# apple/ml-pgdvs

Measured on AMD Instinct MI355X. Metric: novel-view frames/s at 1080p x 24 src frames; achieved HBM GB/s vs gfx950 peak, higher is better.
Workload: dtype f32

## Files before the change

ml-pgdvs_amd/csrc/raster.hip:

```cpp
#include <cstdlib>

#include "common.h"
#include "raster_cam.h"

namespace pgdvs {

constexpr int kTile = 16;

struct TileBox {
  int tx0, tx1, ty0, ty1;
};

__device__ __forceinline__ TileBox tile_box(const RasterCam &rc, float3 p, float radius, int H,
                                            int W, int ntx, int nty) {
  TileBox b;
  b.tx0 = 1;
  b.tx1 = 0;
  b.ty0 = 1;
  b.ty1 = 0;
  if (!(p.z >= 0.0f) || !isfinite(p.x) || !isfinite(p.y)) return b;
  float offx = rc.range_x / 2.0f, offy = rc.range_y / 2.0f;
  float xc = (float)(W - 1) - ((p.x + offx) * (float)W - offx) / rc.range_x;
  float yc = (float)(H - 1) - ((p.y + offy) * (float)H - offy) / rc.range_y;
  float rpx = radius * (float)W / rc.range_x + 0.0625f;
// ... 157 lines not shown
  for (int64_t i = lo + threadIdx.x; i < hi; i += kBinThreads) {
    const float cur[3] = {nxt[0], nxt[1], nxt[2]};
    if (i + kBinThreads < hi && i + kBinThreads < n) {
      const float *X = pts + (i + kBinThreads) * pts_stride;
      nxt[0] = X[0]; nxt[1] = X[1]; nxt[2] = X[2];
    }
    TileBox b;
    b.tx0 = 1; b.tx1 = 0; b.ty0 = 1; b.ty1 = 0;
    float pz = 0.0f;
    if (i < n) {
      float3 p = point_to_ndc(rc, cur[0], cur[1], cur[2]);
      b = tile_box(rc, p, radius, H, W, ntx, nty);
      pz = p.z + 0.0f;
    }
    int nx = 2, ny = 2;
    if (!box2) {
      nx = wave_max_i32_scalar(b.tx1 - b.tx0 + 1);
      ny = wave_max_i32_scalar(b.ty1 - b.ty0 + 1);
    }
    for (int jy = 0; jy < ny; ++jy)
      for (int jx = 0; jx < nx; ++jx) {
        int tx = b.tx0 + jx, ty = b.ty0 + jy;
        int t = (tx <= b.tx1 && ty <= b.ty1) ? ty * ntx + tx : -1;
        if (tile_bound != nullptr && t >= 0 && pz > tile_bound[t]) t = -1;
        if (local)
          wave_tile_count_lds(s_tab, t);
        else
          wave_tile_count(tile_count, t);
      }
  }
  if (local) {
    __syncthreads();
    for (int t = threadIdx.x; t < ntiles; t += kBinThreads) {
      const int v = s_tab[t];
      if (v) __hip_atomic_fetch_add(&tile_count[t], v, __ATOMIC_RELAXED, __HIP_MEMORY_SCOPE_AGENT);
    }
  }
}

__global__ void __launch_bounds__(1024)
raster_scan_kernel(const int32_t *__restrict__ counts, int n, int32_t *__restrict__ offsets, const int32_t *__restrict__ run_flag) {
  __shared__ int wave_sums[1024 / kWave];
  if (run_flag != nullptr && *run_flag == 0) return;
  constexpr int kPer = 8;
  const int lane = threadIdx.x & 63, wave = threadIdx.x >> 6;
  int carry = 0;
  for (int start = 0; start < n; start += 1024 * kPer) {
    const int i0 = start + (int)threadIdx.x * kPer;
    int v[kPer], s = 0;
#pragma unroll
    for (int k = 0; k < kPer; ++k) {
      v[k] = i0 + k < n ? counts[i0 + k] : 0;
      s += v[k];
    }
    int x = s;
    for (int off = 1; off < 64; off <<= 1) {
      const int y = __shfl_up(x, off, 64);
      if (lane >= off) x += y;
    }
    if (lane == 63) wave_sums[wave] = x;
    __syncthreads();
    int run = carry + x - s, total = 0;
#pragma unroll
    for (int w = 0; w < 1024 / kWave; ++w) {
      if (w < wave) run += wave_sums[w];
      total += wave_sums[w];
    }
#pragma unroll
    for (int k = 0; k < kPer; ++k) {
      if (i0 + k < n) offsets[i0 + k] = run;
      run += v[k];
    }
    carry += total;
    __syncthreads();
  }
  if (threadIdx.x == 0) offsets[n] = carry;
}

constexpr int kFillPer = 4;
constexpr int kFillThreads = 256;
constexpr int kFillMaxSpan = 2;

constexpr int kFillTouchCap = 1024;

__device__ __forceinline__ int wave_tile_reserve_lds(int *s_tab, int t, unsigned short *s_touch, int *s_ntouch) {
  const int lane = threadIdx.x & 63;
  RunInfo r = wave_runs(t);
  int base = 0;
  if (r.is_leader && t >= 0) {
    base = atomicAdd(&s_tab[t], r.length);
    if (base == 0) {
      const int at = atomicAdd(s_ntouch, 1);
      if (at < kFillTouchCap) s_touch[at] = (unsigned short)t;
    }
  }
  base = __shfl(base, r.leader, 64);
  return base + (lane - r.leader);
}

template <int kSlots>
__global__ void __launch_bounds__(kFillThreads)
raster_fill_kernel(const float *__restrict__ pts, int64_t pts_stride, int64_t n_host, const int64_t *__restrict__ n_dev,
                   const float *__restrict__ cam, float radius, int H, int W, int ntx, int nty,
                   const int32_t *__restrict__ offsets,
                   int32_t *__restrict__ cursor, float4 *__restrict__ lists,
                   int64_t list_capacity, const float *__restrict__ tile_bound, int64_t gate_rows,
                   int seg, int32_t *__restrict__ overflow, int32_t *__restrict__ status, const int32_t *__restrict__ run_flag) {
  __shared__ int s_tab[kSlots];
  __shared__ unsigned short s_touch[kFillTouchCap];
  __shared__ int s_ntouch;
  static_assert(kSlots <= 65536, "tile numbers in the touched list are 16 bits wide");
  int n_touched = kFillTouchCap + 1;
  if (run_flag != nullptr && *run_flag == 0) return;
  int64_t n = n_dev ? *n_dev : n_host;
  if (status != nullptr && blockIdx.x == 0 && threadIdx.x == 0) *status = n > n_host ? 1 : (n < 0 ? 2 : 0);
  if (seg > 0 && blockIdx.x == 0 && threadIdx.x == 0) overflow[1] = 1;
  n = n > n_host ? n_host : (n < 0 ? 0 : n);
  if (n < gate_rows) tile_bound = nullptr;
  RasterCam rc = make_raster_cam(cam, H, W);
  const int ntiles = ntx * nty;
  const bool local = ntiles <= kSlots && tile_box_within_2x2(rc, radius, H, W);
  constexpr int64_t kChunk = (int64_t)kFillThreads * kFillPer;
  for (int64_t c0 = (int64_t)blockIdx.x * kChunk; c0 < n; c0 += (int64_t)gridDim.x * kChunk) {
    int t0[kFillPer], span[kFillPer];
    float ex[kFillPer], ey[kFillPer], ez[kFillPer];
#pragma unroll
    for (int u = 0; u < kFillPer; ++u) {
      const int64_t i = c0 + (int64_t)u * kFillThreads + threadIdx.x;
      const float *X = pts + (i < n ? i : n - 1) * pts_stride;
      ex[u] = X[0];
      ey[u] = X[1];
      ez[u] = X[2];
    }
    if (local) {
      if (n_touched <= kFillTouchCap) {
        for (int k = threadIdx.x; k < n_touched; k += kFillThreads) s_tab[s_touch[k]] = 0;
      } else {
        for (int t = threadIdx.x; t < ntiles; t += kFillThreads) s_tab[t] = 0;
      }
      if (threadIdx.x == 0) s_ntouch = 0;
      __syncthreads();
    }
#pragma unroll
    for (int u = 0; u < kFillPer; ++u) {
      const int64_t i = c0 + (int64_t)u * kFillThreads + threadIdx.x;
      TileBox b;
      b.tx0 = 1; b.tx1 = 0; b.ty0 = 1; b.ty1 = 0;
      if (i < n) {
        const float3 q = point_to_ndc(rc, ex[u], ey[u], ez[u]);
        b = tile_box(rc, q, radius, H, W, ntx, nty);
        ex[u] = q.x;
        ey[u] = q.y;
        ez[u] = q.z + 0.0f;
      }
      t0[u] = b.ty0 * ntx + b.tx0;
      span[u] = (b.tx1 - b.tx0 + 1) | ((b.ty1 - b.ty0 + 1) << 16);
      if (tile_bound != nullptr && local) {
        unsigned behind = 0;
#pragma unroll
        for (int jy = 0; jy < kFillMaxSpan; ++jy)
#pragma unroll
          for (int jx = 0; jx < kFillMaxSpan; ++jx)
            if (jx < (span[u] & 0xff) && jy < (span[u] >> 16) && ez[u] > tile_bound[t0[u] + jy * ntx + jx]) behind |= 1u << (8 + jy * 2 + jx);
        span[u] |= (int)behind;
      }
    }
    if (local) {
      unsigned rank[kFillPer][kFillMaxSpan];
#pragma unroll
      for (int u = 0; u < kFillPer; ++u) {
#pragma unroll
        for (int jy = 0; jy < kFillMaxSpan; ++jy) {
          rank[u][jy] = 0;
#pragma unroll
          for (int jx = 0; jx < kFillMaxSpan; ++jx) {
            const int t = (jx < (span[u] & 0xff) && jy < (span[u] >> 16) && !((span[u] >> (8 + jy * 2 + jx)) & 1))
                              ? t0[u] + jy * ntx + jx : -1;
            rank[u][jy] |= ((unsigned)wave_tile_reserve_lds(s_tab, t, s_touch, &s_ntouch) & 0xffffu) << (16 * jx);
          }
        }
      }
      static_assert(kChunk <= 65536, "ranks are packed in 16 bits");
      __syncthreads();
      n_touched = s_ntouch;
      if (n_touched <= kFillTouchCap) {
        for (int kb = threadIdx.x; kb < n_touched; kb += kFillThreads * 4) {
          int t[4], v[4], r[4];
#pragma unroll
          for (int k = 0; k < 4; ++k) {
            const int idx = kb + k * kFillThreads;
            t[k] = idx < n_touched ? (int)s_touch[idx] : -1;
            v[k] = t[k] >= 0 ? s_tab[t[k]] : 0;
          }
#pragma unroll
          for (int k = 0; k < 4; ++k) {
            r[k] = 0;
            if (t[k] >= 0) {
              if (seg > 0) {
                const int at = atomicAdd(&cursor[t[k]], v[k]);
                if (at + v[k] > seg) atomicOr(overflow, 1);
                r[k] = t[k] * seg + at;
              } else {
                r[k] = offsets[t[k]] + atomicAdd(&cursor[t[k]], v[k]);
              }
            }
          }
#pragma unroll
          for (int k = 0; k < 4; ++k)
            if (t[k] >= 0) s_tab[t[k]] = r[k];
        }
      } else
      for (int tb = threadIdx.x; tb < ntiles; tb += kFillThreads * 4) {
        int v[4], r[4];
#pragma unroll
        for (int k = 0; k < 4; ++k) {
          const int t = tb + k * kFillThreads;
          v[k] = t < ntiles ? s_tab[t] : 0;
        }
#pragma unroll
        for (int k = 0; k < 4; ++k) {
          const int t = tb + k * kFillThreads;
          if (seg > 0) {
            const int at = v[k] ? atomicAdd(&cursor[t], v[k]) : 0;
            if (at + v[k] > seg) atomicOr(overflow, 1);
            r[k] = t * seg + at;
          } else {
            r[k] = v[k] ? offsets[t] + atomicAdd(&cursor[t], v[k]) : 0;
          }
        }
#pragma unroll
        for (int k = 0; k < 4; ++k)
          if (v[k]) s_tab[tb + k * kFillThreads] = r[k];
      }
      __syncthreads();
#pragma unroll
      for (int u = 0; u < kFillPer; ++u) {
        const int64_t i = c0 + (int64_t)u * kFillThreads + threadIdx.x;
        const float4 ent = make_float4(ex[u], ey[u], __int_as_float((int)i), ez[u]);
#pragma unroll
        for (int jy = 0; jy < kFillMaxSpan; ++jy)
#pragma unroll
          for (int jx = 0; jx < kFillMaxSpan; ++jx)
            if (jx < (span[u] & 0xff) && jy < (span[u] >> 16) && !((span[u] >> (8 + jy * 2 + jx)) & 1)) {
              const int t = t0[u] + jy * ntx + jx;
              const int64_t pos = (int64_t)s_tab[t] + (int)((rank[u][jy] >> (16 * jx)) & 0xffffu);
              if (pos < (seg > 0 ? (int64_t)(t + 1) * seg : list_capacity)) lists[pos] = ent;
            }
      }
      __syncthreads();
    } else {
#pragma unroll
      for (int u = 0; u < kFillPer; ++u) {
        const int64_t i = c0 + (int64_t)u * kFillThreads + threadIdx.x;
        const float4 ent = make_float4(ex[u], ey[u], __int_as_float((int)i), ez[u]);
        const int nx = wave_max_i32_scalar(span[u] & 0xffff), ny = wave_max_i32_scalar(span[u] >> 16);
        for (int jy = 0; jy < ny; ++jy)
          for (int jx = 0; jx < nx; ++jx) {
            int t = (jx < (span[u] & 0xffff) && jy < (span[u] >> 16)) ? t0[u] + jy * ntx + jx : -1;
            if (tile_bound != nullptr && t >= 0 && ez[u] > tile_bound[t]) t = -1;
            const int slot = wave_tile_reserve(cursor, t);
            if (t >= 0) {
              if (seg > 0) {
                if (slot < seg)
                  lists[(int64_t)t * seg + slot] = ent;
                else
                  atomicOr(overflow, 1);
              } else {
                const int64_t pos = (int64_t)offsets[t] + slot;
                if (pos < list_capacity) lists[pos] = ent;
              }
            }
          }
      }
    }
  }
}

template <int K>
struct TopK {
  unsigned long long key[K];
  static constexpr unsigned long long kEmpty = ~0ull;
  __device__ __forceinline__ void init() {
#pragma unroll
    for (int k = 0; k < K; ++k) key[k] = kEmpty;
  }
  __device__ __forceinline__ bool has(int k) const { return key[k] != kEmpty; }
  __device__ __forceinline__ int id(int k) const { return (int)(unsigned)(key[k] & 0xffffffffull); }
  __device__ __forceinline__ float z(int k) const { return __uint_as_float((unsigned)(key[k] >> 32)); }
  __device__ __forceinline__ void insert_below_last(unsigned long long kk) {
    bool c[K];
#pragma unroll
    for (int k = 0; k < K - 1; ++k) c[k] = kk < key[k];
    c[K - 1] = true;
#pragma unroll
    for (int k = K - 1; k > 0; --k) key[k] = c[k - 1] ? key[k - 1] : (c[k] ? kk : key[k]);
    key[0] = c[0] ? kk : key[0];
  }
};

constexpr int kSortCap = 2048;
constexpr int kSortCapLong = 4096;
constexpr int kSortBuckets = 1024;
constexpr int kSortMaxBucket = 64;

template <int K>
__device__ __forceinline__ void rank_insert(float (&key)[K], float r) {
#pragma unroll
  for (int k = K - 1; k > 0; --k) key[k] = __builtin_amdgcn_fmed3f(key[k - 1], key[k], r);
  asm("v_min_f32 %0, %1, %2" : "=v"(key[0]) : "v"(key[0]), "v"(r));
}

__device__ __forceinline__ float readlane_f(float v, int lane) {
  return __int_as_float(__builtin_amdgcn_readlane(__float_as_int(v), lane));
}

template <int K, int kCap, bool kFrag>
__global__ void __launch_bounds__(256, kCap <= kSortCap ? (kFrag ? 4 : 5) : 2)
raster_tile_kernel(const float4 *__restrict__ lists, const int32_t *__restrict__ offsets, int64_t list_capacity,
                   const float4 *__restrict__ seg_lists, const int32_t *__restrict__ seg_count, int seg,
                   const int32_t *__restrict__ seg_overflow, int pass,
                   const float *__restrict__ feat, int64_t feat_stride, float radius, int H, int W,
                   int ntx, int nty, int tiles_per_xcd, int64_t *__restrict__ idx_out,
                   float *__restrict__ zbuf_out, float *__restrict__ dist_out,
                   float *__restrict__ rgb_out, int rgb_planar, float *__restrict__ mask_out, int32_t *__restrict__ stats) {
  constexpr int kSortPerThread = kCap / 256;
  __shared__ uint2 s_buf[kCap];
  uint2 *s_kz = s_buf;
  float2 *s_xy = reinterpret_cast<float2 *>(s_buf);
  __shared__ unsigned s_id[kCap];
  __shared__ unsigned s_zr[kFrag ? kCap : 1];
  __shared__ float4 s_wave[4][68];
  unsigned *s_cnt = reinterpret_cast<unsigned *>(&s_wave[0][0]);
  static_assert(kSortBuckets * 4 <= 4 * 68 * 16, "the counters alias the strips");
  static_assert(kCap * (kFrag ? 16 : 12) + 4 * 68 * 16 + 128 <= (kCap <= kSortCap ? (kFrag ? 40960 : 32768) : 81920),
                "four / five (two) workgroups per CU");
  static_assert(kCap % 256 == 0 && kCap <= 4096, "every thread owns kCap / 256 entries; positions are packed in 12 bits");
  __shared__ unsigned s_red[12];
  __shared__ int s_flag;
  const int ntiles = ntx * nty;
  (void)tiles_per_xcd;
  const int tile = blockIdx.x;
  if (tile >= ntiles) return;
  const int ty = tile / ntx, tx = tile - ty * ntx;
  const int tid = threadIdx.x, lane = tid & 63, wave = tid >> 6;
  const int lx = (wave & 1) * 8 + (lane & 7), ly = (wave >> 1) * 8 + (lane >> 3);
  const int xi = tx * kTile + lx, yi = ty * kTile + ly;
  const bool inside = xi < W && yi < H;
  const float range_x = W > H ? 2.0f * (float)W / (float)H : 2.0f;
  const float range_y = H > W ? 2.0f * (float)H / (float)W : 2.0f;
  const float xf = inside ? pix_to_ndc(W - 1 - xi, W, range_x) : __builtin_nanf("");
  const float yf = pix_to_ndc(H - 1 - yi, H, range_y);
  const float r2 = radius * radius;
  const int qx0 = tx * kTile + (wave & 1) * 8, qy0 = ty * kTile + (wave >> 1) * 8;
  const float margin = radius * 1.001f + 1e-6f;
  const float bx_hi = pix_to_ndc(W - 1 - qx0, W, range_x) + margin;
  const float bx_lo = pix_to_ndc(W - 1 - (qx0 + 7), W, range_x) - margin;
  const float by_hi = pix_to_ndc(H - 1 - qy0, H, range_y) + margin;
  const float by_lo = pix_to_ndc(H - 1 - (qy0 + 7), H, range_y) - margin;
  const bool direct = seg > 0 && *seg_overflow == 0;
  int64_t beg, end;
  if (direct) {
    beg = (int64_t)tile * seg;
    end = beg + seg_count[tile];
  } else {
    beg = offsets[tile];
    end = offsets[tile + 1];
    if (end > list_capacity) end = list_capacity;
  }
  const int64_t n64 = end > beg ? end - beg : 0;
  const float4 *__restrict__ L = (direct ? seg_lists : lists) + beg;

  bool has[K];
  int rid[K];
  float rz[K], rd2[K];
#pragma unroll
  for (int k = 0; k < K; ++k) {
    has[k] = false;
    rid[k] = -1;
    rz[k] = -1.0f;
    rd2[k] = -1.0f;
  }

  if ((pass == 1 && n64 > kSortCap) || (pass == 2 && n64 <= kSortCap)) return;
  bool sorted_path = n64 > 0 && n64 <= kCap;
  if (sorted_path) {
    const int n = (int)n64;
    float4 ent[kSortPerThread];
#pragma unroll
    for (int k = 0; k < kSortPerThread; ++k) {
      const int e = tid + k * 256;
      ent[k] = L[e < n ? e : n - 1];
    }
    unsigned zmn = 0xffffffffu, zmx = 0u;
#pragma unroll
    for (int k = 0; k < kSortPerThread; ++k) {
      const unsigned zb = __float_as_uint(ent[k].w);
      zmn = zb < zmn ? zb : zmn;
      zmx = zb > zmx ? zb : zmx;
    }
#pragma unroll
    for (int off = 32; off > 0; off >>= 1) {
      const unsigned a = __shfl_xor(zmn, off, 64), b = __shfl_xor(zmx, off, 64);
      zmn = a < zmn ? a : zmn;
      zmx = b > zmx ? b : zmx;
    }
    if (lane == 0) {
      s_red[wave] = zmn;
      s_red[4 + wave] = zmx;
    }
#pragma unroll
    for (int j = 0; j < kSortBuckets / 256; ++j) s_cnt[tid + j * 256] = 0u;
    if (tid == 0) s_flag = 0;
    __syncthreads();
#pragma unroll
    for (int w = 0; w < 4; ++w) {
      zmn = s_red[w] < zmn ? s_red[w] : zmn;
      zmx = s_red[4 + w] > zmx ? s_red[4 + w] : zmx;
    }
    const float scale = (float)kSortBuckets / ((float)(zmx - zmn) + 1.0f);
    unsigned pos[kSortPerThread];
#pragma unroll
    for (int k = 0; k < kSortPerThread; ++k) {
      pos[k] = 0u;
      if (k * 256 < n) {
        const int e = tid + k * 256;
        if (e < n) {
          const unsigned zb = __float_as_uint(ent[k].w);
          unsigned b = (unsigned)((float)(zb - zmn) * scale);
          b = b < (unsigned)kSortBuckets - 1u ? b : (unsigned)kSortBuckets - 1u;
          pos[k] = (b << 12) | atomicAdd(&s_cnt[b], 1u);
        }
      }
    }
    __syncthreads();
    {
      unsigned c[kSortBuckets / 256], tot = 0u, mx = 0u;
#pragma unroll
      for (int j = 0; j < kSortBuckets / 256; ++j) {
        c[j] = s_cnt[tid * (kSortBuckets / 256) + j];
        mx = c[j] > mx ? c[j] : mx;
        tot += c[j];
      }
      if (mx > (unsigned)kSortMaxBucket) s_flag = 1;
      unsigned incl = tot;
#pragma unroll
      for (int off = 1; off < 64; off <<= 1) {
        const unsigned y = __shfl_up(incl, off, 64);
        if (lane >= off) incl += y;
      }
      if (lane == 63) s_red[8 + wave] = incl;
      __syncthreads();
      unsigned base = incl - tot;
#pragma unroll
      for (int w = 0; w < 4; ++w)
        if (w < wave) base += s_red[8 + w];
#pragma unroll
      for (int j = 0; j < kSortBuckets / 256; ++j) {
        s_cnt[tid * (kSortBuckets / 256) + j] = base;
        base += c[j];
      }
    }
    __syncthreads();
    sorted_path = s_flag == 0;
    if (!sorted_path && tid == 0) atomicAdd(&stats[0], 1);
    if (sorted_path) {
#pragma unroll
      for (int k = 0; k < kSortPerThread; ++k) {
        if (k * 256 < n) {
          const int e = tid + k * 256;
          if (e < n) {
            const float4 q = ent[k];
            const unsigned b = pos[k] >> 12;
            const unsigned p = s_cnt[b] + (pos[k] & 0xfffu);
            s_kz[p] = make_uint2(__float_as_uint(q.w), __float_as_uint(q.z));
            pos[k] = (b << 12) | p;
          }
        }
      }
      __syncthreads();
#pragma unroll
      for (int k = 0; k < kSortPerThread; ++k) {
        if (k * 256 < n) {
          const int e = tid + k * 256;
          if (e < n) {
            const unsigned b = pos[k] >> 12, p = pos[k] & 0xfffu;
            const unsigned bs = s_cnt[b], be = b + 1u < (unsigned)kSortBuckets ? s_cnt[b + 1u] : (unsigned)n;
            const uint2 me = s_kz[p];
            unsigned r = bs;
            uint2 o[4];
#pragma unroll
            for (int j = 0; j < 4; ++j) o[j] = s_kz[bs + j < (unsigned)n ? bs + j : (unsigned)n - 1u];
#pragma unroll
            for (int j = 0; j < 4; ++j)
              r += (bs + j < be) & ((o[j].x < me.x) | ((o[j].x == me.x) & (o[j].y < me.y))) ? 1u : 0u;
            for (unsigned j = bs + 4u; j < be; ++j) {
              const uint2 oj = s_kz[j];
              r += (oj.x < me.x) | ((oj.x == me.x) & (oj.y < me.y)) ? 1u : 0u;
            }
            pos[k] = r;
          }
        }
      }
      __syncthreads();
#pragma unroll
      for (int k = 0; k < kSortPerThread; ++k) {
        if (k * 256 < n) {
          const int e = tid + k * 256;
          if (e < n) {
            const float4 q = ent[k];
            s_xy[pos[k]] = make_float2(q.x, q.y);
            s_id[pos[k]] = __float_as_uint(q.z);
            if (kFrag) s_zr[pos[k]] = __float_as_uint(q.w);
          }
        }
      }
      __syncthreads();
      float key[K];
#pragma unroll
      for (int k = 0; k < K; ++k) key[k] = __builtin_inff();
      float4 *strip = s_wave[wave];
      for (int base = 0; base < n; base += 64) {
        const unsigned long long open = __ballot(inside && key[K - 1] == __builtin_inff());
        if (open == 0ull) break;
        const int r_lo = __builtin_ctzll(open) >> 3, r_hi = (63 - __builtin_clzll(open)) >> 3;
        unsigned cols = (unsigned)(open | (open >> 32));
        cols |= cols >> 16;
        cols = (cols | (cols >> 8)) & 0xffu;
        const int c_lo = __builtin_ctz(cols), c_hi = 31 - __builtin_clz(cols);
        const float ox_hi = readlane_f(xf, __builtin_ctzll(open & (0x0101010101010101ull << c_lo)));
        const float ox_lo = readlane_f(xf, __builtin_ctzll(open & (0x0101010101010101ull << c_hi)));
        const float oy_hi = readlane_f(yf, r_lo * 8), oy_lo = readlane_f(yf, r_hi * 8);
        const int e = base + lane;
        const float2 c = s_xy[e < n ? e : 0];
        const float ex = fmaxf(fmaxf(ox_lo - c.x, c.x - ox_hi), 0.0f), ey = fmaxf(fmaxf(oy_lo - c.y, c.y - oy_hi), 0.0f);
        const bool in = e < n && ex * ex + ey * ey <= margin * margin;
        const unsigned long long mask = __ballot(in);
        if (!mask) continue;
        const int cnt = (int)__popcll(mask);
        if (in) strip[__popcll(mask & ((1ull << lane) - 1ull))] = make_float4(c.x, c.y, (float)e, 0.f);
        if (lane < 3) strip[cnt + lane] = make_float4(__builtin_inff(), __builtin_inff(), __builtin_inff(), 0.f);
        __builtin_amdgcn_wave_barrier();
        float4 p[4], pn[4];
#pragma unroll
        for (int u = 0; u < 4; ++u) p[u] = strip[u];
        for (int j = 0; j < cnt; j += 4) {
#pragma unroll
          for (int u = 0; u < 4; ++u) pn[u] = strip[(j + 4 + u) & 63];
#pragma unroll
          for (int u = 0; u < 4; ++u) {
            const float dx = p[u].x - xf, dy = p[u].y - yf;
            const float d2 = dx * dx + dy * dy;
            rank_insert<K>(key, d2 < r2 ? p[u].z : __builtin_inff());
          }
#pragma unroll
          for (int u = 0; u < 4; ++u) p[u] = pn[u];
        }
        __builtin_amdgcn_wave_barrier();
      }
#pragma unroll
      for (int k = 0; k < K; ++k) {
        if (key[k] != __builtin_inff()) {
          const int r = (int)key[k];
          const float2 c = s_xy[r];
          const float dx = c.x - xf, dy = c.y - yf;
          has[k] = true;
          rid[k] = (int)s_id[r];
          rz[k] = kFrag ? __uint_as_float(s_zr[kFrag ? r : 0]) : 0.0f;
          rd2[k] = dx * dx + dy * dy;
        }
      }
    }
  }
  if (!sorted_path && n64 > 0) {
    __syncthreads();
    float4 *s_pt = reinterpret_cast<float4 *>(s_xy);
    TopK<K> q;
    q.init();
    for (int64_t base = 0; base < n64; base += 256) {
      const int64_t e = base + tid;
      __syncthreads();
      if (e < n64) s_pt[tid] = L[e];
      __syncthreads();
      const int m = (int)((n64 - base) < 256 ? (n64 - base) : 256);
      for (int sub = 0; sub < m; sub += 64) {
        const int zcull = wave_max_i32_scalar(inside ? (q.has(K - 1) ? (int)(q.key[K - 1] >> 32) : 0x7fffffff) : 0);
        const float4 c = s_pt[(sub + lane) & 255];
        const bool hit = (sub + lane) < m && c.x >= bx_lo && c.x <= bx_hi && c.y >= by_lo && c.y <= by_hi &&
                         __float_as_int(c.w) <= zcull;
        const unsigned long long mask = __ballot(hit);
        if (!mask) continue;
        const int cnt = (int)__popcll(mask);
        float4 *strip = s_wave[wave];
        if (hit) strip[__popcll(mask & ((1ull << lane) - 1ull))] = c;
        if (lane < 3) strip[cnt + lane] = make_float4(__builtin_inff(), __builtin_inff(), 0.f, 0.f);
        __builtin_amdgcn_wave_barrier();
        for (int j = 0; j < cnt; j += 4) {
          float4 p[4];
#pragma unroll
          for (int u = 0; u < 4; ++u) p[u] = strip[j + u];
#pragma unroll
          for (int u = 0; u < 4; ++u) {
            const float dx = p[u].x - xf, dy = p[u].y - yf;
            const float d2 = dx * dx + dy * dy;
            const unsigned long long kk =
                ((unsigned long long)__float_as_uint(p[u].w) << 32) | __float_as_uint(p[u].z);
            if ((d2 < r2) & (kk < q.key[K - 1])) q.insert_below_last(kk);
          }
        }
        __builtin_amdgcn_wave_barrier();
      }
    }
#pragma unroll
    for (int k = 0; k < K; ++k) {
      if (q.has(k)) {
        has[k] = true;
        rid[k] = q.id(k);
        rz[k] = q.z(k);
      }
    }
    for (int64_t base = 0; base < n64; base += 256) {
      const int64_t e = base + tid;
      __syncthreads();
      if (e < n64) s_pt[tid] = L[e];
      __syncthreads();
      const int m = (int)((n64 - base) < 256 ? (n64 - base) : 256);
      for (int j = 0; j < m; ++j) {
        const float4 c = s_pt[j];
        const int id = __float_as_int(c.z);
#pragma unroll
        for (int k = 0; k < K; ++k)
          if (has[k] && rid[k] == id) {
            const float dx = c.x - xf, dy = c.y - yf;
            rd2[k] = dx * dx + dy * dy;
          }
      }
    }
  }
  if (!inside) return;
  const size_t pix = (size_t)yi * W + xi;
  float t = 0.0f;
#pragma unroll
  for (int k = 0; k < K; ++k)
    if (has[k]) t = t + (1.0f - rd2[k] / r2);
  t = t > 1e-4f ? t : 1e-4f;
  float acc[3] = {0.f, 0.f, 0.f}, ones = 0.0f;
#pragma unroll
  for (int k = 0; k < K; ++k) {
    if (idx_out) idx_out[pix * K + k] = has[k] ? (int64_t)rid[k] : (int64_t)-1;
    if (zbuf_out) zbuf_out[pix * K + k] = has[k] ? rz[k] : -1.0f;
    if (dist_out) dist_out[pix * K + k] = rd2[k];
    if (has[k]) {
      float w = 1.0f - rd2[k] / r2;
      ones = ones + w * 1.0f / t;
      if (rgb_out) {
        const float *f = feat + (int64_t)rid[k] * feat_stride;
#pragma unroll
        for (int c = 0; c < 3; ++c) acc[c] = acc[c] + w * f[c] / t;
      }
    }
  }
  if (rgb_out) {
    if (rgb_planar) {
      const size_t P = (size_t)H * W;
#pragma unroll
      for (int c = 0; c < 3; ++c) rgb_out[c * P + pix] = acc[c];
    } else {
#pragma unroll
      for (int c = 0; c < 3; ++c) rgb_out[pix * 3 + c] = acc[c];
    }
  }
  if (mask_out) mask_out[pix] = ones > 0.0f ? 1.0f : 0.0f;
}

__global__ void raster_status_kernel(const int64_t *__restrict__ n_dev, int32_t *__restrict__ status) {
  if (threadIdx.x == 0) *status = (n_dev && *n_dev > 0) ? 1 : ((n_dev && *n_dev < 0) ? 2 : 0);
}

static int64_t max_tiles_per_point(float radius, int H, int W) {
  float range_x = W > H ? 2.0f * (float)W / (float)H : 2.0f;
  float range_y = H > W ? 2.0f * (float)H / (float)W : 2.0f;
  double wx = 2.0 * ((double)radius * W / range_x + 1.5) + 2.0;
  double wy = 2.0 * ((double)radius * H / range_y + 1.5) + 2.0;
  int64_t nx = (int64_t)(wx / kTile) + 2, ny = (int64_t)(wy / kTile) + 2;
  int64_t ntx = cdiv(W, kTile), nty = cdiv(H, kTile);
  if (nx > ntx) nx = ntx;
  if (ny > nty) ny = nty;
  return nx * ny;
}

constexpr double kSegLayoutDensity = 2.2;
constexpr int kSegEntries = 4096;
struct RasterWs {
  int32_t *tile_count, *cursor, *offsets;
  int32_t *seg_cursor;
  float4 *seg_lists;
  int seg_entries;
  int32_t *stats;
  unsigned *zmin;
  float *tile_bound;
  float4 *lists;
  int64_t list_capacity;
  int64_t total_bytes;
};

static RasterWs raster_ws_layout(void *base, int64_t n, int H, int W, float radius) {
  RasterWs w;
  int64_t ntiles = cdiv(W, kTile) * cdiv(H, kTile);
  char *p = reinterpret_cast<char *>(base);
  int64_t off = 0;
  w.tile_count = reinterpret_cast<int32_t *>(p + off);
  off += align_up(ntiles * 4, 256);
  w.cursor = reinterpret_cast<int32_t *>(p + off);
  off += align_up(ntiles * 4, 256);
  w.seg_cursor = reinterpret_cast<int32_t *>(p + off);
  off += align_up(ntiles * 4, 256);
  w.stats = reinterpret_cast<int32_t *>(p + off);
  off += 256;
  w.offsets = reinterpret_cast<int32_t *>(p + off);
  off += align_up((ntiles + 1) * 4, 256);
  w.tile_bound = reinterpret_cast<float *>(p + off);
  off += align_up(ntiles * 4, 256);
  w.zmin = reinterpret_cast<unsigned *>(p + off);
  off += align_up((int64_t)H * W * 4, 256);
  w.list_capacity = (n > 0 ? n : 1) * max_tiles_per_point(radius, H, W);
  w.lists = reinterpret_cast<float4 *>(p + off);
  off += align_up(w.list_capacity * 16, 256);
  w.seg_lists = nullptr;
  w.seg_entries = 0;
  if (ntiles >= 16 && n > 0 && (double)n < kSegLayoutDensity * (double)H * (double)W) {
    int64_t se = align_up(2 * cdiv(w.list_capacity, ntiles), 256);
    se = se < 256 ? 256 : (se > kSegEntries ? kSegEntries : se);
    if (ntiles * se * 16 <= (2ll << 30)) {
      w.seg_entries = (int)se;
      w.seg_lists = reinterpret_cast<float4 *>(p + off);
      off += align_up(ntiles * se * 16, 256);
    }
  }
  w.total_bytes = off;
  return w;
}

__global__ void __launch_bounds__(1024) raster_counters_kernel(const int32_t *__restrict__ offsets, int ntiles,
                                                                const int32_t *__restrict__ stats, int64_t *__restrict__ out,
                                                                const int32_t *__restrict__ seg_cursor, int seg) {
  __shared__ int s_max[16], s_long[16];
  __shared__ long long s_tot[16];
  const bool direct = seg > 0 && seg_cursor != nullptr && stats[2] != 0 && stats[1] == 0;
  int mx = 0, nlong = 0;
  long long tot = 0;
  for (int t = threadIdx.x; t < ntiles; t += 1024) {
    const int n = direct ? seg_cursor[t] : offsets[t + 1] - offsets[t];
    tot += n;
    mx = n > mx ? n : mx;
    nlong += n > kSortCap ? 1 : 0;
  }
  for (int off = 32; off > 0; off >>= 1) {
    const int a = __shfl_xor(mx, off, 64);
    mx = a > mx ? a : mx;
    nlong += __shfl_xor(nlong, off, 64);
    tot += __shfl_xor(tot, off, 64);
  }
  if ((threadIdx.x & 63) == 0) {
    s_max[threadIdx.x >> 6] = mx;
    s_long[threadIdx.x >> 6] = nlong;
    s_tot[threadIdx.x >> 6] = tot;
  }
  __syncthreads();
  if (threadIdx.x == 0) {
    int m = 0, l = 0;
    long long tt = 0;
    for (int w = 0; w < 16; ++w) {
      m = s_max[w] > m ? s_max[w] : m;
      l += s_long[w];
      tt += s_tot[w];
    }
    out[0] = tt;
    out[1] = m;
    out[2] = l;
    out[3] = stats[0];
  }
}

void raster_counters(const void *workspace, int64_t n_rows, int H, int W, float radius, int64_t *out_dev, hipStream_t st) {
  const RasterWs ws = raster_ws_layout(const_cast<void *>(workspace), n_rows, H, W, radius);
  const int ntiles = (int)(cdiv(W, kTile) * cdiv(H, kTile));
  PGDVS_LAUNCH("raster_counters", raster_counters_kernel, dim3(1), dim3(1024), 0, st, (const int32_t *)ws.offsets, ntiles,
               (const int32_t *)ws.stats, out_dev, (const int32_t *)ws.seg_cursor, ws.seg_entries);
}

}

using namespace pgdvs;

namespace pgdvs {
void raster_counter_block(void *workspace, int64_t n_rows, int H, int W, float radius, void **block, int64_t *bytes) {
  const RasterWs ws = raster_ws_layout(workspace, n_rows, H, W, radius);
  *block = ws.tile_count;
  *bytes = (int64_t)((char *)ws.offsets - (char *)ws.tile_count);
}
}
static int points_raster_impl(const float *pts, int64_t pts_stride, const float *feat, int64_t feat_stride, int64_t n_points,
                              const int64_t *n_points_dev, int32_t *status_dev, const float *cam_tgt, float radius, int K,
                              int H, int W, int64_t *idx, float *zbuf, float *dist2, float *rgb, int rgb_planar, float *mask,
                              void *workspace, int64_t workspace_bytes, pgdvs_stream_t stream, bool counters_cleared);
namespace pgdvs {
int points_raster_bounded_cleared(const float *pts, int64_t pts_stride, const float *feat, int64_t feat_stride, int64_t n_points,
                                  const int64_t *n_points_dev, int64_t row_bound, int32_t *status_dev, const float *cam_tgt,
                                  float radius, int K, int H, int W, float *rgb, int rgb_planar, float *mask, void *workspace,
                                  int64_t workspace_bytes, pgdvs_stream_t stream, bool counters_cleared) {
  PGDVS_REQUIRE(row_bound >= 0 && status_dev && n_points >= 0, "points_raster_bounded_cleared: bad arguments");
  if (n_points_dev == nullptr && n_points > row_bound) {
    set_error("pgdvs_points_raster_bounded: %lld rows given (host count) but the row bound is %lld", (long long)n_points,
              (long long)row_bound);
    return PGDVS_ERR_INVALID;
  }
  return points_raster_impl(pts, pts_stride, feat, feat_stride, n_points < row_bound ? n_points : row_bound, n_points_dev,
                            status_dev, cam_tgt, radius, K, H, W, nullptr, nullptr, nullptr, rgb, rgb_planar, mask, workspace,
                            workspace_bytes, stream, counters_cleared);
}
}

PGDVS_API int64_t pgdvs_points_raster_workspace_bytes(int64_t n_points, int H, int W, float radius) {
  if (n_points < 0 || H <= 0 || W <= 0) return -1;
  const RasterWs w = raster_ws_layout(nullptr, n_points, H, W, radius);
  if (w.list_capacity >= (1ll << 31)) {
    set_error("pgdvs_points_raster: %lld points x this radius exceeds the 2^31 tile-list entries supported", (long long)n_points);
    return PGDVS_ERR_UNSUPPORTED;
  }
  return w.total_bytes;
}

template <int K>
static void launch_tile(dim3 grid, hipStream_t st, const RasterWs &ws, const float *feat,
                        int64_t feat_stride, float radius, int H, int W, int ntx, int nty,
                        int tiles_per_xcd, int64_t *idx, float *zbuf, float *dist2, float *rgb,
                        int rgb_planar, float *mask, bool long_lists, int seg) {
  const float4 *sl = (const float4 *)ws.seg_lists;
  const int32_t *sc = (const int32_t *)ws.seg_cursor, *so = (const int32_t *)(ws.stats + 1);
  if (zbuf != nullptr) {
    PGDVS_LAUNCH("raster_tile", (raster_tile_kernel<K, kSortCap, true>), grid, dim3(256), 0, st, (const float4 *)ws.lists,
                 (const int32_t *)ws.offsets, ws.list_capacity, sl, sc, seg, so, long_lists ? 1 : 0, feat, feat_stride, radius, H, W, ntx, nty,
                 tiles_per_xcd, idx, zbuf, dist2, rgb, rgb_planar, mask, ws.stats);
  } else {
    PGDVS_LAUNCH("raster_tile", (raster_tile_kernel<K, kSortCap, false>), grid, dim3(256), 0, st, (const float4 *)ws.lists,
                 (const int32_t *)ws.offsets, ws.list_capacity, sl, sc, seg, so, long_lists ? 1 : 0, feat, feat_stride, radius, H, W, ntx, nty,
                 tiles_per_xcd, idx, zbuf, dist2, rgb, rgb_planar, mask, ws.stats);
  }
  if (long_lists) {
    PGDVS_LAUNCH("raster_tile_long", (raster_tile_kernel<K, kSortCapLong, true>), grid, dim3(256), 0, st, (const float4 *)ws.lists,
                 (const int32_t *)ws.offsets, ws.list_capacity, sl, sc, seg, so, 2, feat, feat_stride, radius, H, W, ntx, nty, tiles_per_xcd, idx, zbuf,
                 dist2, rgb, rgb_planar, mask, ws.stats);
  }
}

static int points_raster_impl(const float *pts, int64_t pts_stride, const float *feat, int64_t feat_stride, int64_t n_points,
                              const int64_t *n_points_dev, int32_t *status_dev, const float *cam_tgt, float radius, int K,
                              int H, int W, int64_t *idx, float *zbuf, float *dist2, float *rgb, int rgb_planar, float *mask,
                              void *workspace, int64_t workspace_bytes, pgdvs_stream_t stream, bool counters_cleared = false);

PGDVS_API int pgdvs_points_raster(const float *pts, int64_t pts_stride, const float *feat,
                                  int64_t feat_stride, int64_t n_points,
                                  const int64_t *n_points_dev, const float *cam_tgt, float radius,
                                  int K, int H, int W, int64_t *idx, float *zbuf, float *dist2,
                                  float *rgb, int rgb_planar, float *mask, void *workspace,
                                  int64_t workspace_bytes, pgdvs_stream_t stream) {
  return points_raster_impl(pts, pts_stride, feat, feat_stride, n_points, n_points_dev, nullptr, cam_tgt, radius, K, H, W, idx,
                            zbuf, dist2, rgb, rgb_planar, mask, workspace, workspace_bytes, stream);
}

PGDVS_API int pgdvs_points_raster_bounded(const float *pts, int64_t pts_stride, const float *feat, int64_t feat_stride,
                                          int64_t n_points, const int64_t *n_points_dev, int64_t row_bound,
                                          int32_t *status_dev, const float *cam_tgt, float radius, int K, int H, int W,
                                          int64_t *idx, float *zbuf, float *dist2, float *rgb, int rgb_planar, float *mask,
                                          void *workspace, int64_t workspace_bytes, pgdvs_stream_t stream) {
  PGDVS_REQUIRE(row_bound >= 0 && status_dev, "pgdvs_points_raster_bounded: bad row_bound / null status_dev");
  PGDVS_REQUIRE(n_points >= 0, "pgdvs_points_raster_bounded: bad n_points");
  if (n_points_dev == nullptr && n_points > row_bound) {
    set_error("pgdvs_points_raster_bounded: %lld rows given (host count) but the row bound is %lld", (long long)n_points,
              (long long)row_bound);
    return PGDVS_ERR_INVALID;
  }
  return points_raster_impl(pts, pts_stride, feat, feat_stride, n_points < row_bound ? n_points : row_bound, n_points_dev,
                            status_dev, cam_tgt, radius, K, H, W, idx, zbuf, dist2, rgb, rgb_planar, mask, workspace,
                            workspace_bytes, stream);
}

static int points_raster_impl(const float *pts, int64_t pts_stride, const float *feat, int64_t feat_stride, int64_t n_points,
                              const int64_t *n_points_dev, int32_t *status_dev, const float *cam_tgt, float radius, int K,
                              int H, int W, int64_t *idx, float *zbuf, float *dist2, float *rgb, int rgb_planar, float *mask,
                              void *workspace, int64_t workspace_bytes, pgdvs_stream_t stream, bool counters_cleared) {
  PGDVS_REQUIRE(H > 0 && W > 0 && (int64_t)H * W < (1ll << 31), "pgdvs_points_raster: bad H/W");
  PGDVS_REQUIRE(n_points >= 0 && n_points < (1ll << 31), "pgdvs_points_raster: bad n_points");
  PGDVS_REQUIRE(cam_tgt && (n_points == 0 || pts) && pts_stride >= 3, "pgdvs_points_raster: bad points");
  PGDVS_REQUIRE(!rgb || n_points == 0 || (feat && feat_stride >= 3), "pgdvs_points_raster: rgb output needs features");
  PGDVS_REQUIRE(radius > 0.0f, "pgdvs_points_raster: radius must be > 0");
  if (K < 1 || K > kRasterMaxK) {
    set_error("pgdvs_points_raster: points_per_pixel must be in [1, %d]", kRasterMaxK);
    return PGDVS_ERR_UNSUPPORTED;
  }
  RasterWs ws = raster_ws_layout(workspace, n_points, H, W, radius);
  if (ws.list_capacity >= (1ll << 31)) {
    set_error("pgdvs_points_raster: %lld points x %lld tiles per point exceeds the 2^31 tile-list entries supported",
              (long long)n_points, (long long)(ws.list_capacity / (n_points > 0 ? n_points : 1)));
    return PGDVS_ERR_UNSUPPORTED;
  }
  if (!workspace || workspace_bytes < ws.total_bytes) {
    set_error("pgdvs_points_raster: workspace too small (%lld < %lld)", (long long)workspace_bytes,
              (long long)ws.total_bytes);
    return PGDVS_ERR_WORKSPACE;
  }
  hipStream_t st = as_stream(stream);
  const int ntx = (int)cdiv(W, kTile), nty = (int)cdiv(H, kTile), ntiles = ntx * nty;
  if (!counters_cleared) {
    hipError_t e = hipMemsetAsync(ws.tile_count, 0, (size_t)((char *)ws.offsets - (char *)ws.tile_count), st);
    if (e != hipSuccess) {
      set_error("points_raster memset: %s", hipGetErrorString(e));
      return PGDVS_ERR_LAUNCH;
    }
  }
  const bool small_table = ntiles <= kBinSlots / 2;
  const float *tile_bound = nullptr;
  int64_t gate_rows = 0;
  {
    const double density = (double)option_float(options().raster_bound_density);
    const float px_per_ndc = (float)(W < H ? W : H) / 2.0f;
    const float rpx = radius * px_per_ndc;
    const int b = rpx >= 5.05f ? 4 : (rpx >= 2.25f ? 2 : 0);
    gate_rows = (int64_t)(density * (double)H * (double)W);
    if (n_points > 0 && n_points >= gate_rows && b != 0 && K <= b * b) {
      const int64_t n16 = cdiv((int64_t)H * W * 4, 16);
      PGDVS_LAUNCH("raster_zmin_init", raster_zmin_init_kernel, dim3((unsigned)(cdiv(n16, 256) < 2048 ? cdiv(n16, 256) : 2048)), dim3(256),
                   0, st, n_points, n_points_dev, gate_rows, reinterpret_cast<uint4 *>(ws.zmin), n16);
      const unsigned gz = (unsigned)(cdiv(n_points, 256) < 4096 ? cdiv(n_points, 256) : 4096);
      PGDVS_LAUNCH("raster_zmin", raster_zmin_kernel, dim3(gz), dim3(256), 0, st, pts, pts_stride, n_points, n_points_dev, gate_rows,
                   cam_tgt, H, W, ws.zmin);
      if (b == 4) {
        PGDVS_LAUNCH("raster_bound", raster_bound_kernel<4>, dim3((unsigned)ntiles), dim3(256), 0, st, (const unsigned *)ws.zmin,
                     n_points, n_points_dev, gate_rows, H, W, ntx, K, ws.tile_bound);
      } else {
        PGDVS_LAUNCH("raster_bound", raster_bound_kernel<2>, dim3((unsigned)ntiles), dim3(256), 0, st, (const unsigned *)ws.zmin,
                     n_points, n_points_dev, gate_rows, H, W, ntx, K, ws.tile_bound);
      }
      tile_bound = ws.tile_bound;
    }
  }
  if (n_points == 0 && status_dev != nullptr) {
    PGDVS_LAUNCH("raster_status", raster_status_kernel, dim3(1), dim3(64), 0, st, n_points_dev, status_dev);
  }
  const int seg = (n_points > 0 && n_points < gate_rows && ws.seg_lists != nullptr) ? ws.seg_entries : 0;
  const int32_t *run_flag = seg > 0 ? ws.stats + 1 : nullptr;
  const int64_t fill_chunks = cdiv(n_points, (int64_t)kFillThreads * kFillPer);
  const unsigned g_fill = (unsigned)(fill_chunks < 4096 ? fill_chunks : 4096);
  if (seg > 0) {
    if (small_table) {
      PGDVS_LAUNCH("raster_fill", raster_fill_kernel<kBinSlots / 2>, dim3(g_fill), dim3(kFillThreads), 0, st, pts, pts_stride, n_points, n_points_dev,
                   cam_tgt, radius, H, W, ntx, nty, (const int32_t *)nullptr, ws.seg_cursor, ws.seg_lists, ws.list_capacity, tile_bound, gate_rows,
                   seg, ws.stats + 1, status_dev, (const int32_t *)nullptr);
    } else {
      PGDVS_LAUNCH("raster_fill", raster_fill_kernel<kBinSlots>, dim3(g_fill), dim3(kFillThreads), 0, st, pts, pts_stride, n_points, n_points_dev,
                   cam_tgt, radius, H, W, ntx, nty, (const int32_t *)nullptr, ws.seg_cursor, ws.seg_lists, ws.list_capacity, tile_bound, gate_rows,
                   seg, ws.stats + 1, status_dev, (const int32_t *)nullptr);
    }
  }
  if (n_points > 0) {
    unsigned g = (unsigned)(cdiv(n_points, kBinThreads) < 512 ? cdiv(n_points, kBinThreads) : 512);
    if (seg > 0 && g > 256) g = 256;
    if (small_table) {
      PGDVS_LAUNCH(seg > 0 ? "raster_exact_count" : "raster_project_count", raster_project_count_kernel<kBinSlots / 2>, dim3(g), dim3(kBinThreads), 0, st, pts,
                   pts_stride, n_points, n_points_dev, cam_tgt, radius, H, W, ntx, nty, ws.tile_count, status_dev, tile_bound, gate_rows, run_flag);
    } else {
      PGDVS_LAUNCH(seg > 0 ? "raster_exact_count" : "raster_project_count", raster_project_count_kernel<kBinSlots>, dim3(g), dim3(kBinThreads), 0, st, pts,
                   pts_stride, n_points, n_points_dev, cam_tgt, radius, H, W, ntx, nty, ws.tile_count, status_dev, tile_bound, gate_rows, run_flag);
    }
  }
  PGDVS_LAUNCH(seg > 0 ? "raster_exact_scan" : "raster_scan", raster_scan_kernel, dim3(1), dim3(1024), 0, st, ws.tile_count, ntiles, ws.offsets, run_flag);
  if (n_points > 0) {
    const unsigned g_exact_fill = seg > 0 && g_fill > 256 ? 256u : g_fill;
    if (small_table) {
      PGDVS_LAUNCH(seg > 0 ? "raster_exact_fill" : "raster_fill", raster_fill_kernel<kBinSlots / 2>, dim3(g_exact_fill), dim3(kFillThreads), 0, st, pts, pts_stride, n_points, n_points_dev, cam_tgt,
                   radius, H, W, ntx, nty, (const int32_t *)ws.offsets, ws.cursor, ws.lists, ws.list_capacity, tile_bound, gate_rows,
                   0, (int32_t *)nullptr, (int32_t *)nullptr, run_flag);
    } else {
      PGDVS_LAUNCH(seg > 0 ? "raster_exact_fill" : "raster_fill", raster_fill_kernel<kBinSlots>, dim3(g_exact_fill), dim3(kFillThreads), 0, st, pts, pts_stride, n_points, n_points_dev, cam_tgt,
                   radius, H, W, ntx, nty, (const int32_t *)ws.offsets, ws.cursor, ws.lists, ws.list_capacity, tile_bound, gate_rows,
                   0, (int32_t *)nullptr, (int32_t *)nullptr, run_flag);
    }
  }
  const int tiles_per_xcd = (int)cdiv(ntiles, 8);
  dim3 grid((unsigned)ntiles);
  const bool long_lists = n_points > 0 && n_points >= gate_rows;
#define PGDVS_TILE_CASE(KK)                                                                      \
  case KK:                                                                                       \
    launch_tile<KK>(grid, st, ws, feat, feat_stride, radius, H, W, ntx, nty, tiles_per_xcd, idx, \
                    zbuf, dist2, rgb, rgb_planar, mask, long_lists, seg);                        \
    break;
  switch (K) {
    PGDVS_TILE_CASE(1)
    PGDVS_TILE_CASE(2)
    PGDVS_TILE_CASE(3)
    PGDVS_TILE_CASE(4)
    PGDVS_TILE_CASE(5)
    PGDVS_TILE_CASE(6)
    PGDVS_TILE_CASE(7)
    PGDVS_TILE_CASE(8)
  }
#undef PGDVS_TILE_CASE
  return check_launch("points_raster");
}
```

Baseline: 1290.

## Rank and rasterize depth-sorted entries slice by slice with early exit

The bucketed depth sort used to compute final ranks for every tile entry before rasterizing. Now entries are grouped into depth slices of about 512 aligned to bucket boundaries. Each slice is ranked, scattered and rasterized in turn, and the block stops once every pixel has K hits. This skips ranking work for far entries, at the cost of extra block barriers per slice and more per-thread state. It also drops the unused tiles_per_xcd parameter and adds slice statistics counters.

```diff
diff --git a/ml-pgdvs_amd/csrc/raster.hip b/ml-pgdvs_amd/csrc/raster.hip
--- a/ml-pgdvs_amd/csrc/raster.hip
+++ b/ml-pgdvs_amd/csrc/raster.hip
@@ -483,6 +483,14 @@
 constexpr int kSortCapLong = 4096;
 constexpr int kSortBuckets = 1024;
 constexpr int kSortMaxBucket = 64;
+#ifndef PGDVS_RASTER_SLICE
+#define PGDVS_RASTER_SLICE 512
+#endif
+constexpr int kSlice = PGDVS_RASTER_SLICE;
+constexpr int kSliceShift = __builtin_ctz(kSlice);
+constexpr int kSlicePerThread = (kSlice + kSortMaxBucket - 1 + 255) / 256;
+static_assert((kSlice & (kSlice - 1)) == 0 && kSlice >= 2 * kSortMaxBucket,
+              "a bucket's slice is its start >> kSliceShift; bucket starts lie closer than a slice is long: no slice is empty");
 
 template <int K>
 __device__ __forceinline__ void rank_insert(float (&key)[K], float r) {
@@ -501,7 +509,7 @@
                    const float4 *__restrict__ seg_lists, const int32_t *__restrict__ seg_count, int seg,
                    const int32_t *__restrict__ seg_overflow, int pass,
                    const float *__restrict__ feat, int64_t feat_stride, float radius, int H, int W,
-                   int ntx, int nty, int tiles_per_xcd, int64_t *__restrict__ idx_out,
+                   int ntx, int nty, int64_t *__restrict__ idx_out,
                    float *__restrict__ zbuf_out, float *__restrict__ dist_out,
                    float *__restrict__ rgb_out, int rgb_planar, float *__restrict__ mask_out, int32_t *__restrict__ stats) {
   constexpr int kSortPerThread = kCap / 256;
@@ -513,13 +521,13 @@
   __shared__ float4 s_wave[4][68];
   unsigned *s_cnt = reinterpret_cast<unsigned *>(&s_wave[0][0]);
   static_assert(kSortBuckets * 4 <= 4 * 68 * 16, "the counters alias the strips");
-  static_assert(kCap * (kFrag ? 16 : 12) + 4 * 68 * 16 + 128 <= (kCap <= kSortCap ? (kFrag ? 40960 : 32768) : 81920),
+  static_assert(kCap * (kFrag ? 16 : 12) + 4 * 68 * 16 + 64 + 8 * (kCap / kSlice) <= (kCap <= kSortCap ? (kFrag ? 40960 : 32768) : 81920),
                 "four / five (two) workgroups per CU");
   static_assert(kCap % 256 == 0 && kCap <= 4096, "every thread owns kCap / 256 entries; positions are packed in 12 bits");
   __shared__ unsigned s_red[12];
   __shared__ int s_flag;
+  __shared__ unsigned s_hi[kCap / kSlice], s_open[kCap / kSlice], s_nsl;
   const int ntiles = ntx * nty;
-  (void)tiles_per_xcd;
   const int tile = blockIdx.x;
   if (tile >= ntiles) return;
   const int ty = tile / ntx, tx = tile - ty * ntx;
@@ -592,6 +600,7 @@
 #pragma unroll
     for (int j = 0; j < kSortBuckets / 256; ++j) s_cnt[tid + j * 256] = 0u;
     if (tid == 0) s_flag = 0;
+    if (tid < kCap / kSlice) s_open[tid] = 0u;
     __syncthreads();
 #pragma unroll
     for (int w = 0; w < 4; ++w) {
@@ -637,8 +646,13 @@
         if (w < wave) base += s_red[8 + w];
 #pragma unroll
       for (int j = 0; j < kSortBuckets / 256; ++j) {
+        const unsigned st = base;
         s_cnt[tid * (kSortBuckets / 256) + j] = base;
         base += c[j];
+        if (c[j] != 0u && (base == (unsigned)n || (base >> kSliceShift) != (st >> kSliceShift))) {
+          s_hi[st >> kSliceShift] = base;
+          if (base == (unsigned)n) s_nsl = (st >> kSliceShift) + 1u;
+        }
       }
     }
     __syncthreads();
@@ -650,93 +664,111 @@
         if (k * 256 < n) {
           const int e = tid + k * 256;
           if (e < n) {
-            const float4 q = ent[k];
-            const unsigned b = pos[k] >> 12;
-            const unsigned p = s_cnt[b] + (pos[k] & 0xfffu);
-            s_kz[p] = make_uint2(__float_as_uint(q.w), __float_as_uint(q.z));
-            pos[k] = (b << 12) | p;
+            const unsigned b = pos[k] >> 12, a = pos[k] & 0xfffu;
+            const unsigned bs = s_cnt[b], be = b + 1u < (unsigned)kSortBuckets ? s_cnt[b + 1u] : (unsigned)n;
+            s_kz[bs + a] = make_uint2(__float_as_uint(ent[k].w), __float_as_uint(ent[k].z));
+            s_id[bs + a] = (unsigned)e | (a << 12) | ((be - bs - 1u) << 18);
           }
         }
       }
       __syncthreads();
-#pragma unroll
-      for (int k = 0; k < kSortPerThread; ++k) {
-        if (k * 256 < n) {
-          const int e = tid + k * 256;
-          if (e < n) {
-            const unsigned b = pos[k] >> 12, p = pos[k] & 0xfffu;
-            const unsigned bs = s_cnt[b], be = b + 1u < (unsigned)kSortBuckets ? s_cnt[b + 1u] : (unsigned)n;
-            const uint2 me = s_kz[p];
-            unsigned r = bs;
-            uint2 o[4];
-#pragma unroll
-            for (int j = 0; j < 4; ++j) o[j] = s_kz[bs + j < (unsigned)n ? bs + j : (unsigned)n - 1u];
-#pragma unroll
-            for (int j = 0; j < 4; ++j)
-              r += (bs + j < be) & ((o[j].x < me.x) | ((o[j].x == me.x) & (o[j].y < me.y))) ? 1u : 0u;
-            for (unsigned j = bs + 4u; j < be; ++j) {
-              const uint2 oj = s_kz[j];
-              r += (oj.x < me.x) | ((oj.x == me.x) & (oj.y < me.y)) ? 1u : 0u;
+      const int nsl = (int)s_nsl;
+      float key[K];
+#pragma unroll
+      for (int k = 0; k < K; ++k) key[k] = __builtin_inff();
+      float4 *strip = s_wave[wave];
+      int lo = 0, sl = 0;
+      for (;;) {
+        const int hi = (int)s_hi[sl];
+        unsigned rk[kSlicePerThread];
+        uint2 me[kSlicePerThread];
+        float2 pxy[kSlicePerThread];
+#pragma unroll
+        for (int i = 0; i < kSlicePerThread; ++i) {
+          rk[i] = 0xffffffffu;
+          me[i] = make_uint2(0u, 0u);
+          pxy[i] = make_float2(0.f, 0.f);
+          if (i * 256 < hi - lo) {
+            const int p = lo + tid + i * 256;
+            if (p < hi) {
+              const unsigned w = s_id[p];
+              me[i] = s_kz[p];
+              pxy[i] = *reinterpret_cast<const float2 *>(L + (w & 0xfffu));
+              const unsigned bs = (unsigned)p - ((w >> 12) & 63u), be = bs + ((w >> 18) & 63u) + 1u;
+              unsigned r = bs;
+              uint2 o[4];
+#pragma unroll
+              for (int j = 0; j < 4; ++j) o[j] = s_kz[bs + j < (unsigned)n ? bs + j : (unsigned)n - 1u];
+#pragma unroll
+              for (int j = 0; j < 4; ++j)
+                r += (bs + j < be) & ((o[j].x < me[i].x) | ((o[j].x == me[i].x) & (o[j].y < me[i].y))) ? 1u : 0u;
+              for (unsigned j = bs + 4u; j < be; ++j) {
+                const uint2 oj = s_kz[j];
+                r += (oj.x < me[i].x) | ((oj.x == me[i].x) & (oj.y < me[i].y)) ? 1u : 0u;
+              }
+              rk[i] = r;
             }
-            pos[k] = r;
           }
         }
-      }
-      __syncthreads();
-#pragma unroll
-      for (int k = 0; k < kSortPerThread; ++k) {
-        if (k * 256 < n) {
-          const int e = tid + k * 256;
-          if (e < n) {
-            const float4 q = ent[k];
-            s_xy[pos[k]] = make_float2(q.x, q.y);
-            s_id[pos[k]] = __float_as_uint(q.z);
-            if (kFrag) s_zr[pos[k]] = __float_as_uint(q.w);
+        __syncthreads();
+#pragma unroll
+        for (int i = 0; i < kSlicePerThread; ++i) {
+          if (rk[i] != 0xffffffffu) {
+            s_xy[rk[i]] = pxy[i];
+            s_id[rk[i]] = me[i].y;
+            if (kFrag) s_zr[rk[i]] = me[i].x;
           }
         }
-      }
-      __syncthreads();
-      float key[K];
-#pragma unroll
-      for (int k = 0; k < K; ++k) key[k] = __builtin_inff();
-      float4 *strip = s_wave[wave];
-      for (int base = 0; base < n; base += 64) {
-        const unsigned long long open = __ballot(inside && key[K - 1] == __builtin_inff());
-        if (open == 0ull) break;
-        const int r_lo = __builtin_ctzll(open) >> 3, r_hi = (63 - __builtin_clzll(open)) >> 3;
-        unsigned cols = (unsigned)(open | (open >> 32));
-        cols |= cols >> 16;
-        cols = (cols | (cols >> 8)) & 0xffu;
-        const int c_lo = __builtin_ctz(cols), c_hi = 31 - __builtin_clz(cols);
-        const float ox_hi = readlane_f(xf, __builtin_ctzll(open & (0x0101010101010101ull << c_lo)));
-        const float ox_lo = readlane_f(xf, __builtin_ctzll(open & (0x0101010101010101ull << c_hi)));
-        const float oy_hi = readlane_f(yf, r_lo * 8), oy_lo = readlane_f(yf, r_hi * 8);
-        const int e = base + lane;
-        const float2 c = s_xy[e < n ? e : 0];
-        const float ex = fmaxf(fmaxf(ox_lo - c.x, c.x - ox_hi), 0.0f), ey = fmaxf(fmaxf(oy_lo - c.y, c.y - oy_hi), 0.0f);
-        const bool in = e < n && ex * ex + ey * ey <= margin * margin;
-        const unsigned long long mask = __ballot(in);
-        if (!mask) continue;
-        const int cnt = (int)__popcll(mask);
-        if (in) strip[__popcll(mask & ((1ull << lane) - 1ull))] = make_float4(c.x, c.y, (float)e, 0.f);
-        if (lane < 3) strip[cnt + lane] = make_float4(__builtin_inff(), __builtin_inff(), __builtin_inff(), 0.f);
-        __builtin_amdgcn_wave_barrier();
-        float4 p[4], pn[4];
-#pragma unroll
-        for (int u = 0; u < 4; ++u) p[u] = strip[u];
-        for (int j = 0; j < cnt; j += 4) {
-#pragma unroll
-          for (int u = 0; u < 4; ++u) pn[u] = strip[(j + 4 + u) & 63];
-#pragma unroll
-          for (int u = 0; u < 4; ++u) {
-            const float dx = p[u].x - xf, dy = p[u].y - yf;
-            const float d2 = dx * dx + dy * dy;
-            rank_insert<K>(key, d2 < r2 ? p[u].z : __builtin_inff());
+        __syncthreads();
+        for (int base = lo; base < hi; base += 64) {
+          const unsigned long long open = __ballot(inside && key[K - 1] == __builtin_inff());
+          if (open == 0ull) break;
+          const int r_lo = __builtin_ctzll(open) >> 3, r_hi = (63 - __builtin_clzll(open)) >> 3;
+          unsigned cols = (unsigned)(open | (open >> 32));
+          cols |= cols >> 16;
+          cols = (cols | (cols >> 8)) & 0xffu;
+          const int c_lo = __builtin_ctz(cols), c_hi = 31 - __builtin_clz(cols);
+          const float ox_hi = readlane_f(xf, __builtin_ctzll(open & (0x0101010101010101ull << c_lo)));
+          const float ox_lo = readlane_f(xf, __builtin_ctzll(open & (0x0101010101010101ull << c_hi)));
+          const float oy_hi = readlane_f(yf, r_lo * 8), oy_lo = readlane_f(yf, r_hi * 8);
+          const int e = base + lane;
+          const float2 c = s_xy[e < hi ? e : lo];
+          const float ex = fmaxf(fmaxf(ox_lo - c.x, c.x - ox_hi), 0.0f), ey = fmaxf(fmaxf(oy_lo - c.y, c.y - oy_hi), 0.0f);
+          const bool in = e < hi && ex * ex + ey * ey <= margin * margin;
+          const unsigned long long mask = __ballot(in);
+          if (!mask) continue;
+          const int cnt = (int)__popcll(mask);
+          if (in) strip[__popcll(mask & ((1ull << lane) - 1ull))] = make_float4(c.x, c.y, (float)e, 0.f);
+          if (lane < 3) strip[cnt + lane] = make_float4(__builtin_inff(), __builtin_inff(), __builtin_inff(), 0.f);
+          __builtin_amdgcn_wave_barrier();
+          float4 p[4], pn[4];
+#pragma unroll
+          for (int u = 0; u < 4; ++u) p[u] = strip[u];
+          for (int j = 0; j < cnt; j += 4) {
+#pragma unroll
+            for (int u = 0; u < 4; ++u) pn[u] = strip[(j + 4 + u) & 63];
+#pragma unroll
+            for (int u = 0; u < 4; ++u) {
+              const float dx = p[u].x - xf, dy = p[u].y - yf;
+              const float d2 = dx * dx + dy * dy;
+              rank_insert<K>(key, d2 < r2 ? p[u].z : __builtin_inff());
+            }
+#pragma unroll
+            for (int u = 0; u < 4; ++u) p[u] = pn[u];
           }
-#pragma unroll
-          for (int u = 0; u < 4; ++u) p[u] = pn[u];
+          __builtin_amdgcn_wave_barrier();
         }
-        __builtin_amdgcn_wave_barrier();
+        if (sl + 1 == nsl) break;
+        const unsigned long long still = __ballot(inside && key[K - 1] == __builtin_inff());
+        if (lane == 0 && still != 0ull) s_open[sl] = 1u;
+        __syncthreads();
+        if (s_open[sl] == 0u) break;
+        lo = hi;
+        ++sl;
+      }
+      if (tid == 0) {
+        atomicAdd(&stats[4], sl + 1);
+        if (nsl - sl - 1 > 0) atomicAdd(&stats[3], nsl - sl - 1);
       }
 #pragma unroll
       for (int k = 0; k < K; ++k) {
@@ -1014,22 +1046,22 @@
 template <int K>
 static void launch_tile(dim3 grid, hipStream_t st, const RasterWs &ws, const float *feat,
                         int64_t feat_stride, float radius, int H, int W, int ntx, int nty,
-                        int tiles_per_xcd, int64_t *idx, float *zbuf, float *dist2, float *rgb,
+                        int64_t *idx, float *zbuf, float *dist2, float *rgb,
                         int rgb_planar, float *mask, bool long_lists, int seg) {
   const float4 *sl = (const float4 *)ws.seg_lists;
   const int32_t *sc = (const int32_t *)ws.seg_cursor, *so = (const int32_t *)(ws.stats + 1);
   if (zbuf != nullptr) {
     PGDVS_LAUNCH("raster_tile", (raster_tile_kernel<K, kSortCap, true>), grid, dim3(256), 0, st, (const float4 *)ws.lists,
                  (const int32_t *)ws.offsets, ws.list_capacity, sl, sc, seg, so, long_lists ? 1 : 0, feat, feat_stride, radius, H, W, ntx, nty,
-                 tiles_per_xcd, idx, zbuf, dist2, rgb, rgb_planar, mask, ws.stats);
+                 idx, zbuf, dist2, rgb, rgb_planar, mask, ws.stats);
   } else {
     PGDVS_LAUNCH("raster_tile", (raster_tile_kernel<K, kSortCap, false>), grid, dim3(256), 0, st, (const float4 *)ws.lists,
                  (const int32_t *)ws.offsets, ws.list_capacity, sl, sc, seg, so, long_lists ? 1 : 0, feat, feat_stride, radius, H, W, ntx, nty,
-                 tiles_per_xcd, idx, zbuf, dist2, rgb, rgb_planar, mask, ws.stats);
+                 idx, zbuf, dist2, rgb, rgb_planar, mask, ws.stats);
   }
   if (long_lists) {
     PGDVS_LAUNCH("raster_tile_long", (raster_tile_kernel<K, kSortCapLong, true>), grid, dim3(256), 0, st, (const float4 *)ws.lists,
-                 (const int32_t *)ws.offsets, ws.list_capacity, sl, sc, seg, so, 2, feat, feat_stride, radius, H, W, ntx, nty, tiles_per_xcd, idx, zbuf,
+                 (const int32_t *)ws.offsets, ws.list_capacity, sl, sc, seg, so, 2, feat, feat_stride, radius, H, W, ntx, nty, idx, zbuf,
                  dist2, rgb, rgb_planar, mask, ws.stats);
   }
 }
@@ -1167,13 +1199,12 @@
                    0, (int32_t *)nullptr, (int32_t *)nullptr, run_flag);
     }
   }
-  const int tiles_per_xcd = (int)cdiv(ntiles, 8);
   dim3 grid((unsigned)ntiles);
   const bool long_lists = n_points > 0 && n_points >= gate_rows;
 #define PGDVS_TILE_CASE(KK)                                                                      \
   case KK:                                                                                       \
-    launch_tile<KK>(grid, st, ws, feat, feat_stride, radius, H, W, ntx, nty, tiles_per_xcd, idx, \
-                    zbuf, dist2, rgb, rgb_planar, mask, long_lists, seg);                        \
+    launch_tile<KK>(grid, st, ws, feat, feat_stride, radius, H, W, ntx, nty, idx, zbuf, dist2,   \
+                    rgb, rgb_planar, mask, long_lists, seg);                                     \
     break;
   switch (K) {
     PGDVS_TILE_CASE(1)
```

Measured after the change: 1186. 8.1% lower.
